# timdestan/go-raytracer

Hardware: AMD Instinct MI355X
Metric: Mrays/s (primary+shadow+reflect) at 4K depth=6; 1/2/4/8-GPU scaling (higher is better)
Workload: dtype f64; 1 GPU; c3: cylinder + cube + sphere (cone substitute) over a reflective plane, 4 lights, 3840x2160, depth 6; width=3840, height=2160, depth=6, lights=4, objects=4, parallelism=rows1-interleaved, frames_in_flight=2, schedule=auto, kernel=specialised, accel=bvh+cull

## Files before the change

### go-raytracer_amd/csrc/rt_kernel.hip

```cpp
#pragma clang fp contract(off)

#include <hip/hip_runtime.h>

#include <dlfcn.h>
#include <errno.h>
#include <fcntl.h>
#include <hip/hiprtc.h>
#include <sys/syscall.h>
#include <sys/wait.h>
#include <unistd.h>

#include <algorithm>
#include <atomic>
#include <chrono>
#include <condition_variable>
#include <cstdlib>
#include <functional>
#include <thread>
#include <cmath>
#include <array>
#include <cstdio>
#include <utility>
#include <cstring>
#include <limits>
// ... 1253 lines not shown
const char* rt_last_error(void) { return g_err.c_str(); }

int rt_create(int device, rt_context** out) {
  if (!out) return fail(RT_E_INVALID, "rt_create: out is NULL");
  *out = nullptr;
  if (device < 0) HIP_TRY(hipGetDevice(&device));
  int ndev = 0;
  HIP_TRY(hipGetDeviceCount(&ndev));
  if (device >= ndev) return fail(RT_E_INVALID, "rt_create: device index out of range");
  DeviceGuard guard(device);
  rt_context* c = new rt_context();
  c->device = device;
  hipDeviceProp_t prop;
  if (hipGetDeviceProperties(&prop, device) != hipSuccess) {
    delete c;
    return fail(RT_E_DEVICE, "hipGetDeviceProperties failed");
  }
  c->cus = prop.multiProcessorCount;
  c->lds_per_cu = (int)prop.maxSharedMemoryPerMultiProcessor;
  c->lds_per_block = (int)prop.sharedMemPerBlock;
  int per_cu = 0;
  if (hipOccupancyMaxActiveBlocksPerMultiprocessor(&per_cu, k_kernels[kernel_index(true, false, false, false, false)], WG, LDS_MAX_BYTES) !=
          hipSuccess || per_cu <= 0)
    per_cu = 2;
  c->grid_lds = c->cus * std::min(per_cu, 8);
  per_cu = 0;
  if (hipOccupancyMaxActiveBlocksPerMultiprocessor(&per_cu, k_kernels[kernel_index(false, false, false, false, false)], WG, 0) != hipSuccess ||
      per_cu <= 0)
    per_cu = 2;
  c->grid_glb = c->cus * std::min(per_cu, 8);
  std::vector<uint64_t> jump(JUMP_ENTRIES * 4);
  {
    typedef unsigned __int128 u128;
    const u128 mul = ((u128)2549297995355413924ULL << 64) | 4865540595714422341ULL;
    const u128 inc = ((u128)6364136223846793005ULL << 64) | 1442695040888963407ULL;
    u128 A = 1, Cc = 0;
    for (int step = 0; step < 2 * JUMP_ENTRIES; step++) {
      if (step % 2 == 0) {
        const int e = step / 2;
        jump[e * 4 + 0] = (uint64_t)(A >> 64);
        jump[e * 4 + 1] = (uint64_t)A;
        jump[e * 4 + 2] = (uint64_t)(Cc >> 64);
        jump[e * 4 + 3] = (uint64_t)Cc;
      }
      A = A * mul;
      Cc = Cc * mul + inc;
    }
  }
  int rc = upload(&c->jump, jump);
  if (rc == RT_OK && hipMalloc((void**)&c->queue, 2 * QSET_ALLOC * sizeof(unsigned int)) != hipSuccess)
    rc = fail(RT_E_NOMEM, "queue alloc");
  if (rc == RT_OK && hipMemset(c->queue, 0, 2 * QSET_ALLOC * sizeof(unsigned int)) != hipSuccess)
    rc = fail(RT_E_DEVICE, "queue memset");
  if (rc == RT_OK && hipMalloc((void**)&c->stats, sizeof(unsigned long long) * 64) != hipSuccess)
    rc = fail(RT_E_NOMEM, "stats alloc");
  if (rc == RT_OK && hipMemset(c->stats, 0, sizeof(unsigned long long) * 64) != hipSuccess)
    rc = fail(RT_E_DEVICE, "stats memset");
  c->stats_parts = c->cus * 8;
  if (rc == RT_OK && hipMalloc((void**)&c->stats_part, sizeof(unsigned long long) * STATS_PART * c->stats_parts) != hipSuccess)
    rc = fail(RT_E_NOMEM, "stats alloc");
  if (rc == RT_OK && hipMemset(c->stats_part, 0, sizeof(unsigned long long) * STATS_PART * c->stats_parts) != hipSuccess)
    rc = fail(RT_E_DEVICE, "stats memset");
  if (rc == RT_OK && (hipEventCreate(&c->ev0) != hipSuccess || hipEventCreate(&c->ev1) != hipSuccess))
    rc = fail(RT_E_DEVICE, "event create");
  if (rc != RT_OK) {
    rt_destroy(c);
    return rc;
  }
  *out = c;
  return RT_OK;
}

void rt_destroy(rt_context* c) {
  if (!c) return;
  DeviceGuard guard(c->device);
  free_scene(c->sc);
  (void)hipFree(c->ssim_buf);
  (void)hipFree(c->jump);
  (void)hipFree(c->queue);
  (void)hipFree(c->stats);
  (void)hipFree(c->stats_part);
  (void)hipFree(c->stack);
  (void)hipFree(c->vm_global);
  clear_orders(c);
  (void)hipFree(c->est);
  (void)hipFree(c->est_stats);
  (void)hipFree(c->gboard);
  (void)hipFree(c->gring);
  (void)hipFree(c->gctl);
  (void)hipFree(c->trace_ws);
  (void)hipFree(c->trace_ticket);
  (void)hipFree(c->cam_buf);
  (void)hipFree(c->cam_adapt);
  if (c->ev0) (void)hipEventDestroy(c->ev0);
  if (c->ev1) (void)hipEventDestroy(c->ev1);
  delete c;
}

static int launch(rt_context* c, int y0, int y1, int trow0, int stride, int ntrows, void* d_rgba, void* stream,
                  bool est);
static int estimate_costs(rt_context* c);
static bool want_order(const rt_context* c);
static int scene_install(rt_context* c, DevScene& s, const std::vector<uint32_t>* costs);

int rt_set_scene(rt_context* c, const rt_scene* in) {
  if (!c || !in) return fail(RT_E_INVALID, "rt_set_scene: NULL argument");
  if (in->width <= 1 || in->height <= 1) return fail(RT_E_INVALID, "rt_set_scene: width/height must be > 1");
  if (in->exp_mode < RT_EXP_AMD64_FMA || in->exp_mode > RT_EXP_PORTABLE)
    return fail(RT_E_INVALID, "rt_set_scene: unknown exp_mode");
// ... 813 lines not shown
      P.bvh_hi[k] = s.bvh_hi[k];
    }
  }

  if (c->launched && st != c->last_stream) HIP_TRY(hipStreamWaitEvent(st, c->ev1, 0));
  c->last_stream = st;
  c->launched = true;
  if (!est) HIP_TRY(hipEventRecord(c->ev0, st));
  const char* blob = s.blob;
  void* args[] = {(void*)&blob, (void*)&P};
  if (spec)
    HIP_TRY(hipModuleLaunchKernel(spec, grid, 1, 1, WG, 1, 1, shmem, st, args, nullptr));
  else
    HIP_TRY(hipLaunchKernel(kfn, dim3(grid), dim3(WG), args, shmem, st));
  HIP_TRY(hipGetLastError());
  c->qset ^= 1;
  HIP_TRY(hipEventRecord(c->ev1, st));
  if (est) return RT_OK;
  c->timed = true;
  c->last_spec = spec != nullptr;
  uint64_t rows = 0;
  if (stride > 0) {
    for (int j = 0; j < ntrows; j++) {
      int r0 = (trow0 + j * stride) * TILE;
      rows += (uint64_t)std::max(0, std::min((int)TILE, s.height - r0));
    }
  } else {
    rows = (uint64_t)(y1 - y0);
  }
  c->primary_pending += (uint64_t)4 * (uint64_t)s.width * rows;
  return RT_OK;
}

static bool want_order(const rt_context* c) {
  static const int env = rt_getenv("RT_TILE_ORDER") ? atoi(rt_getenv("RT_TILE_ORDER")) : 1;
  const DevScene& s = c->sc;
  return env != 0 && c->order_on && s.nobj > 0 && (scene_in_lds(s) || (env == 2 && s.use_bvh));
}

static int estimate_costs(rt_context* c) {
  clear_orders(c);
  if (!want_order(c)) return RT_OK;
  const DevScene& s = c->sc;
  DeviceGuard guard(c->device);
  const size_t n = (size_t)((s.width + TILE - 1) / TILE) * ((s.height + TILE - 1) / TILE);
  if (n > c->est_cap) {
    (void)hipFree(c->est);
    c->est = nullptr;
    c->est_cap = 0;
    HIP_TRY(hipMalloc((void**)&c->est, n * sizeof(unsigned int)));
    c->est_cap = n;
  }
  if (!c->est_stats) {
    HIP_TRY(hipMalloc((void**)&c->est_stats, sizeof(unsigned long long) * 64));
    HIP_TRY(hipMemset(c->est_stats, 0, sizeof(unsigned long long) * 64));
  }
  const auto t0 = std::chrono::steady_clock::now();
  HIP_TRY(hipMemset(c->est, 0, n * sizeof(unsigned int)));
  int rc = launch(c, 0, s.height, 0, 0, 0, nullptr, nullptr, true);
  if (rc != RT_OK) return rc;
  std::vector<uint32_t> cost(n);
  HIP_TRY(hipMemcpy(cost.data(), c->est, n * sizeof(unsigned int), hipMemcpyDeviceToHost));
  unsigned long long wd = 0;
  HIP_TRY(hipMemcpy(&wd, c->est_stats + ST_WATCHDOG, sizeof wd, hipMemcpyDeviceToHost));
  HIP_TRY(hipMemset(c->est_stats, 0, sizeof(unsigned long long) * 64));
  if (wd) return fail(RT_E_DEVICE, "render watchdog in the tile-cost estimate (kernel bug)");
  c->tile_cost.swap(cost);
  c->order_ms = std::chrono::duration<double, std::milli>(std::chrono::steady_clock::now() - t0).count();
  c->timed = false;
  return RT_OK;
}

int rt_set_work_sharing(rt_context* c, int enable) {
  if (!c) return fail(RT_E_INVALID, "rt_set_work_sharing: NULL context");
  if (enable < 0 || enable > RT_SHARE_AUTO) return fail(RT_E_INVALID, "rt_set_work_sharing: unknown mode");
  c->share_mode = enable;
  return c->has_scene ? spec_prepare(c) : RT_OK;
}

int rt_set_tile_order(rt_context* c, int enable) {
  if (!c) return fail(RT_E_INVALID, "rt_set_tile_order: NULL context");
  c->order_on = enable != 0;
  if (!c->has_scene) return RT_OK;
  if (!c->order_on) {
    clear_orders(c);
    return RT_OK;
  }
  return c->tile_cost.empty() ? estimate_costs(c) : RT_OK;
}

int rt_tile_order_info(rt_context* c, int* active, double* estimate_ms) {
  if (!c || !active || !estimate_ms) return fail(RT_E_INVALID, "rt_tile_order_info: NULL argument");
  *active = c->tile_cost.empty() ? 0 : 1;
  *estimate_ms = c->order_ms;
  return RT_OK;
}

int rt_render_rows_async(rt_context* c, int y0, int y1, void* d_rgba, void* stream) {
  if (!c || !c->has_scene) return fail(RT_E_INVALID, "rt_render_rows_async: no scene set");
  if (!d_rgba) return fail(RT_E_INVALID, "rt_render_rows_async: NULL output");
  if (y0 < 0 || y1 > c->sc.height || y1 <= y0) return fail(RT_E_INVALID, "rt_render_rows_async: bad row range");
  return launch(c, y0, y1, 0, 0, 0, d_rgba, stream, false);
}

int rt_render_tile_rows_async(rt_context* c, int trow0, int trow_stride, int ntrows, void* d_rgba, void* stream) {
  if (!c || !c->has_scene) return fail(RT_E_INVALID, "rt_render_tile_rows_async: no scene set");
  if (!d_rgba) return fail(RT_E_INVALID, "rt_render_tile_rows_async: NULL output");
  if (trow0 < 0 || trow_stride <= 0 || ntrows <= 0) return fail(RT_E_INVALID, "rt_render_tile_rows_async: bad tile rows");
  return launch(c, 0, c->sc.height, trow0, trow_stride, ntrows, d_rgba, stream, false);
}


int rt_read_stats(rt_context* c, void* stream, int reset, rt_stats* out) {
  if (!c || !out) return fail(RT_E_INVALID, "rt_read_stats: NULL argument");
  DeviceGuard guard(c->device);
  hipStream_t st = (hipStream_t)stream;
  unsigned long long h[ST_COUNT] = {}, wd = 0;
  std::vector<unsigned long long> part((size_t)STATS_PART * c->stats_parts);
  HIP_TRY(hipMemcpyAsync(part.data(), c->stats_part, part.size() * sizeof(unsigned long long), hipMemcpyDeviceToHost, st));
  HIP_TRY(hipMemcpyAsync(&wd, c->stats + ST_WATCHDOG, sizeof wd, hipMemcpyDeviceToHost, st));
  HIP_TRY(hipStreamSynchronize(st));
  for (int b = 0; b < c->stats_parts; b++)
    for (int k = 0; k < ST_COUNT; k++) h[k] += part[(size_t)b * STATS_PART + k];
  if (wd) {
    HIP_TRY(hipMemsetAsync(c->stats, 0, sizeof(unsigned long long) * 64, st));
    HIP_TRY(hipMemsetAsync(c->stats_part, 0, part.size() * sizeof(unsigned long long), st));
    c->gslots = 0;
    HIP_TRY(hipStreamSynchronize(st));
    c->primary_pending = 0;
    c->launches = 0;
    return fail(RT_E_DEVICE, "render watchdog: " + std::to_string(wd) + " waves stopped unfinished (kernel bug)");
  }
  std::memset(out, 0, sizeof *out);
  uint64_t per_kind[RT_NUM_KINDS] = {0, 0, 0, 0, 0};
  if (c->has_scene)
    for (int k : c->sc.kinds) per_kind[k]++;
  out->primary_rays = c->primary_pending;
  out->secondary_rays = h[ST_TRACED] - c->primary_pending;
  out->shadow_rays = h[ST_SHADOW];
  for (int k = 0; k < RT_NUM_KINDS; k++) {
    out->tests[k] = h[ST_TRACED] * per_kind[k];
    out->shadow_tests[k] = h[ST_STESTS + k];
  }
  out->shaded_hits = h[ST_SHADED];
  out->surface_errors = h[ST_SURFERR];
#ifdef RT_PHASE_TIMING
  {
    unsigned long long ph[N_PHASE];
    HIP_TRY(hipMemcpy(ph, c->stats + ST_PHASE, sizeof ph, hipMemcpyDeviceToHost));
    unsigned long long tot = 0;
    for (int k = 0; k < N_PHASE; k++) tot += ph[k];
    if (tot) {
      static const char* nm[N_PHASE] = {"refill", "gen", "trace_loop", "trace_unwind", "shade_surface",
                                        "light_dirs", "shadow_loops", "lighting", "material", "shade_unwind"};
      fprintf(stderr, "[phase]");
      for (int k = 0; k < N_PHASE; k++) fprintf(stderr, " %s=%.3f", nm[k], (double)ph[k] / (double)tot);
      fprintf(stderr, " total_wave_cycles=%.4g\n", (double)tot);
      unsigned long long bd[8];
      HIP_TRY(hipMemcpy(bd, c->stats + ST_BVHDIAG, sizeof bd, hipMemcpyDeviceToHost));
      if (c->wdiag && c->last_waves > 0) {
        std::vector<unsigned long long> w((size_t)c->last_waves * 4);
        HIP_TRY(hipMemcpy(w.data(), c->wdiag, w.size() * sizeof(unsigned long long), hipMemcpyDeviceToHost));
        std::vector<std::pair<unsigned long long, int>> life;
        for (int i = 0; i < c->last_waves; i++) life.push_back({w[(size_t)i * 4], i});
        std::sort(life.begin(), life.end());
        auto pct = [&](double q) { return (double)life[std::min(life.size() - 1, (size_t)(q * life.size()))].first; };
        fprintf(stderr, "[tail] lifetime p10 %.4g p50 %.4g p90 %.4g p99 %.4g max %.4g;", pct(0.1), pct(0.5), pct(0.9),
                pct(0.99), (double)life.back().first);
        for (int k = 1; k <= 4 && k <= (int)life.size(); k++) {
          const int i = life[life.size() - k].second;
          fprintf(stderr, " [life %.4g chunks %llu last-chunk %.4g]", (double)w[(size_t)i * 4], w[(size_t)i * 4 + 1],
                  (double)w[(size_t)i * 4 + 2]);
        }
        double lc = 0;
        for (int i = 0; i < c->last_waves; i++) lc += (double)w[(size_t)i * 4 + 2];
        fprintf(stderr, " mean last-chunk %.4g\n", lc / c->last_waves);
      }
#ifdef RT_CSG_DIAG
      {
        unsigned long long cd[8] = {0, 0, 0, 0, 0, 0, 0, 0};
        if (hipMemcpyFromSymbol(cd, HIP_SYMBOL(g_csg_diag), sizeof cd) == hipSuccess && cd[0]) {
          fprintf(stderr, "[csg] searches %llu, register-list overflows %llu (%.2f%%), mean live leaves %.2f\n", cd[0],
                  cd[1], 100.0 * cd[1] / cd[0], (double)cd[2] / cd[0]);
          if (cd[6])
            fprintf(stderr,
                    "[csg] group visits %llu: leaf-major iterations %llu (lanes %.1f of 64), lane-major %llu (lanes "
                    "%.1f), lane-leaf candidates %llu\n",
                    cd[6], cd[3], cd[3] ? (double)cd[5] / cd[3] : 0.0, cd[4], cd[4] ? (double)cd[5] / cd[4] : 0.0, cd[5]);
        }
      }
#endif
      {
        unsigned long long sh[6];
        HIP_TRY(hipMemcpy(sh, c->stats + ST_SHDIAG, sizeof sh, hipMemcpyDeviceToHost));
        fprintf(stderr, "[share] posted samples %llu subtrees %llu, claims %llu, reclaims %llu, waits %llu, idle polls %llu\n",
                sh[0], sh[1], sh[2], sh[3], sh[4], sh[5]);
      }
      {
        unsigned long long pd[6];
        HIP_TRY(hipMemcpy(pd, c->stats + ST_PASSDIAG, sizeof pd, hipMemcpyDeviceToHost));
        fprintf(stderr, "[passes] trace %llu (%.1f lanes), shade %llu (%.1f lanes), gen %llu (%.1f lanes)\n", pd[0],
                (double)pd[1] / std::max(1ull, pd[0]), pd[2], (double)pd[3] / std::max(1ull, pd[2]), pd[4],
                (double)pd[5] / std::max(1ull, pd[4]));
        unsigned long long ld[2];
        HIP_TRY(hipMemcpy(ld, c->stats + ST_LANEDIAG, sizeof ld, hipMemcpyDeviceToHost));
        fprintf(stderr, "[lanes] rounds %llu, lanes waiting in S_DONE (finished quad / pair samples) %.2f per round\n", ld[1],
                (double)ld[0] / (double)std::max(1ull, ld[1]));
      }
      unsigned long long steps = 0;
      HIP_TRY(hipMemcpy(&steps, c->stats + ST_CLOCKSTEP, sizeof steps, hipMemcpyDeviceToHost));
      const double nw = std::max(1.0, (double)c->last_waves * c->launches - (double)steps);
      fprintf(stderr, "[waves] lifetime mean %.4g cycles, max %.4g cycles (mean/max %.3f; %llu waves with a clock step left out)\n",
              (double)bd[6] / nw, (double)bd[7], (double)bd[6] / nw / (double)std::max(1ull, bd[7]), steps);
      if (bd[4] + bd[5])
        fprintf(stderr, "[bvh] wave traversals trace=%llu shadow=%llu; nodes/traversal trace=%.1f shadow=%.1f; "
                        "leaves/traversal trace=%.1f shadow=%.1f\n", bd[4], bd[5], (double)bd[0] / (double)std::max(1ull, bd[4]),
                (double)bd[1] / (double)std::max(1ull, bd[5]), (double)bd[2] / (double)std::max(1ull, bd[4]),
                (double)bd[3] / (double)std::max(1ull, bd[5]));
#ifdef RT_EXACT_DIAG
      unsigned long long ex[2 * RT_NUM_KINDS + 2];
      HIP_TRY(hipMemcpy(ex, c->stats + ST_EXDIAG, sizeof ex, hipMemcpyDeviceToHost));
      fprintf(stderr, "[exact] lane tests after culling per kind (trace/shadow):");
      for (int k = 0; k < RT_NUM_KINDS; k++) fprintf(stderr, " k%d=%llu/%llu", k, ex[2 * k], ex[2 * k + 1]);
      fprintf(stderr, "; wave batches trace=%llu shadow=%llu\n", ex[2 * RT_NUM_KINDS], ex[2 * RT_NUM_KINDS + 1]);
#endif
    }
  }
#endif
  float ms = 0.f;
  if (c->timed && hipEventElapsedTime(&ms, c->ev0, c->ev1) == hipSuccess) out->kernel_ms = ms;
  out->devices = 1;
  out->device_kernel_ms[0] = out->kernel_ms;
  if (reset) {
    HIP_TRY(hipMemsetAsync(c->stats, 0, sizeof(unsigned long long) * 64, st));
    HIP_TRY(hipMemsetAsync(c->stats_part, 0, part.size() * sizeof(unsigned long long), st));
    HIP_TRY(hipStreamSynchronize(st));
    c->primary_pending = 0;
    c->launches = 0;
  }
  return RT_OK;
}

int rt_last_kernel_ms(rt_context* c, double* ms_out) {
  if (!c || !ms_out) return fail(RT_E_INVALID, "rt_last_kernel_ms: NULL argument");
  if (!c->timed) return fail(RT_E_INVALID, "rt_last_kernel_ms: nothing rendered yet");
  DeviceGuard guard(c->device);
  HIP_TRY(hipEventSynchronize(c->ev1));
  float ms = 0.f;
  HIP_TRY(hipEventElapsedTime(&ms, c->ev0, c->ev1));
  *ms_out = ms;
  return RT_OK;
}

int rt_debug_run_surface(rt_context* c, int program, int n, const long long* face, const double* u,
                         const double* v, double* out10, int* err) {
  if (!c || !c->has_scene || n <= 0 || !face || !u || !v || !out10 || !err)
    return fail(RT_E_INVALID, "rt_debug_run_surface: bad arguments");
  if (program < 0 || program >= c->sc.num_programs) return fail(RT_E_INVALID, "rt_debug_run_surface: no such program");
  DeviceGuard guard(c->device);
  long long* df = nullptr;
  double *du = nullptr, *dv = nullptr, *dout = nullptr;
  int* derr = nullptr;
  int rc = RT_OK;
  if (hipMalloc((void**)&df, n * sizeof(long long)) != hipSuccess || hipMalloc((void**)&du, n * sizeof(double)) != hipSuccess ||
      hipMalloc((void**)&dv, n * sizeof(double)) != hipSuccess ||
      hipMalloc((void**)&dout, (size_t)n * 10 * sizeof(double)) != hipSuccess ||
      hipMalloc((void**)&derr, n * sizeof(int)) != hipSuccess)
    rc = fail(RT_E_NOMEM, "rt_debug_run_surface: alloc");
  if (rc == RT_OK && (hipMemcpy(df, face, n * sizeof(long long), hipMemcpyHostToDevice) != hipSuccess ||
                      hipMemcpy(du, u, n * sizeof(double), hipMemcpyHostToDevice) != hipSuccess ||
                      hipMemcpy(dv, v, n * sizeof(double), hipMemcpyHostToDevice) != hipSuccess))
    rc = fail(RT_E_DEVICE, "rt_debug_run_surface: copy");
  if (rc == RT_OK) {
    hipLaunchKernelGGL(rt_debug_vm_kernel, dim3((n + 63) / 64), dim3(64), 0, nullptr, (const char*)c->sc.blob,
                       c->sc.off_code, c->sc.off_consts, c->sc.off_entry, program, df, du, dv, dout, derr, n);
    if (hipGetLastError() != hipSuccess || hipDeviceSynchronize() != hipSuccess)
      rc = fail(RT_E_DEVICE, "rt_debug_run_surface: launch");
  }
  if (rc == RT_OK && (hipMemcpy(out10, dout, (size_t)n * 10 * sizeof(double), hipMemcpyDeviceToHost) != hipSuccess ||
                      hipMemcpy(err, derr, n * sizeof(int), hipMemcpyDeviceToHost) != hipSuccess))
    rc = fail(RT_E_DEVICE, "rt_debug_run_surface: copy back");
  (void)hipFree(df);
  (void)hipFree(du);
  (void)hipFree(dv);
  (void)hipFree(dout);
  (void)hipFree(derr);
  return rc;
// ... 11 lines not shown
```

### go-raytracer_amd/csrc/rt_render.h

```cpp
#pragma once
#pragma clang fp contract(off)

#ifndef __HIPCC_RTC__
#include <hip/hip_runtime.h>
#endif

#include "rt_abi.h"
#include "rt_device.h"

#ifndef RT_CULL
#define RT_CULL 1
#endif
#ifndef RT_SHARE
#define RT_SHARE 0
#endif
#ifndef RT_PAIRS
#define RT_PAIRS 0
#endif
#ifndef RT_FAR_SHIFT
#define RT_FAR_SHIFT 1
#endif
#ifndef RT_GS_POLL
#define RT_GS_POLL 3
#endif
#ifndef RT_GS_HELPERS
#define RT_GS_HELPERS 16
#endif
#ifndef RT_SHADE_NUM
#define RT_SHADE_NUM 3
#endif
#ifndef RT_SHADE_DEN
#define RT_SHADE_DEN 4
#endif
#ifdef RT_COST_MAP
#undef RT_SHARE
#define RT_SHARE 0
#endif

#define CULL_AND(a, b) (bool)((int)(bool)(a) & (int)(bool)(b))

using namespace rt;

enum { SF_VM = 1, SF_LDIR = 2, SF_LSPOT = 4 };
#ifdef RT_SPEC_NOBJ
constexpr int spec_kinds[RT_SPEC_NOBJ] = {RT_SPEC_KINDS};
constexpr int spec_kind_mask() {
  int m = 0;
  for (int i = 0; i < RT_SPEC_NOBJ; i++) m |= 1 << spec_kinds[i];
  return m;
}
constexpr int SPEC_KMASK = spec_kind_mask();
constexpr int SPEC_FEAT = RT_SPEC_FEAT;
static_assert(SPEC_KMASK == RT_SPEC_KMASK, "RT_SPEC_KINDS and RT_SPEC_KMASK disagree");
#elif defined(RT_SPEC_KMASK)
constexpr int SPEC_KMASK = RT_SPEC_KMASK;
constexpr int SPEC_FEAT = RT_SPEC_FEAT;
#else
constexpr int SPEC_KMASK = -1;
constexpr int SPEC_FEAT = -1;
#endif
__device__ constexpr bool spec_kind(int k) { return ((SPEC_KMASK >> k) & 1) != 0; }
__device__ constexpr bool spec_feat(int f) { return (SPEC_FEAT & f) != 0; }

enum { GEO = 16, SHD = 32, MAT = 16, LGT = 16, OMAT = 8, GLOB = 16 };
enum { FRAME_FIELDS = 15, CORE = 5, EXT_ROWS = 6, FR_EXT = 3, FR_COL = 11, FR_REFL = 14 };
enum { CHUNK = 64, TILE = 8, WG = 256, WAVES_PER_WG = WG / 64 };
enum { QHEADS = 8 , QSTRIDE = 16  };
static_assert(QHEADS >= 1 && QHEADS <= 32, "QHEADS");
enum { QSTEAL = 1 };
enum { QSET = QHEADS * QSTRIDE ,
       QSET_ALLOC = 32 * QSTRIDE  };
enum { QCHUNK_PIXEL = 64 };
enum { SCH = 32 };
enum { SHADOW_CHECK = 8 };
enum { ST_SHADOW = 0, ST_TRACED = 1, ST_SHADED = 2, ST_SURFERR = 3, ST_STESTS = 4, ST_COUNT = ST_STESTS + RT_NUM_KINDS,
       ST_PHASE = 16, N_PHASE = 10, ST_BVHDIAG = 26, ST_EXDIAG = 34, ST_SHDIAG = 48, ST_PASSDIAG = 54,
       ST_CLOCKSTEP = 60, ST_LANEDIAG = 61 ,
       ST_WATCHDOG = 63,
       STATS_PART = 16  };
enum { SH_POST_S = 0, SH_POST_T = 1, SH_CLAIM = 2, SH_RECLAIM = 3, SH_WAIT = 4, SH_SPIN = 5 };
#ifdef RT_PHASE_TIMING
#define SHDIAG(k) atomicAdd(P.stats + ST_SHDIAG + (k), 1ull)
#else
#define SHDIAG(k) (void)0
#endif
enum { S_IDLE = 0, S_TRACE = 1, S_SHADE = 2, S_DONE = 3 };
enum { LDS_MAX_BYTES = 40 * 1024 };
enum { JUMP_ENTRIES = 20 * 4 };

__device__ __forceinline__ int est_x(int pts, unsigned int k) { return pts == 1 ? TILE / 2 : 2 + 4 * (int)(k & 1u); }
__device__ __forceinline__ int est_y(int pts, unsigned int k) { return pts == 1 ? TILE / 2 : 2 + 4 * (int)((k >> 1) & 1u); }

struct Params {
  int lds_frames_off;
  int lds_levels;
  int lds_full;
  int lds_ext_off;
  int stream_off;
  int qmask_off;
  int jump_off;
  int off_geo, off_shade, off_mats, off_lights, off_kind, off_objmat, off_pref, off_csg, off_code, off_consts,
      off_entry, blob_bytes;
  int lds_vm_off;
  double* vm_global;
  const uint64_t* jump;
  unsigned int* queue;
  unsigned int* queue_next;
  unsigned long long* stats;
  unsigned long long* stats_part;
  unsigned long long* wdiag;
  double* stack;
  uint32_t* out;
  int width, height, depth, nobj, nlights, y0, y1, tiles_x;
  int trow0, trow_stride;
  unsigned int total_slots;
  int frames;
  const float* bvh_nodes;
  const double* bvh_geo;
  const int* planes;
  int nplanes, bvh_stack_off;
  double bvh_lo[3], bvh_hi[3];
  const int* runs;
  int nruns;
  const double* arec;
  const double* urec;
  int cnt_off;
  int kind_mask;
  int board_off;
  uint64_t* gboard;
  uint64_t* gring;
  uint64_t* gctl;
// ... 1297 lines not shown
      pk = lane_ < min(SCH, P.nobj - c0) ? S.kind[c0 + lane_] : 0;
    };
    auto store = [&]() {
#pragma unroll
      for (int q = 0; q < PER; q++) dst[lane_ + q * 64] = pre[q];
      if (lane_ < SCH) skind[lane_] = pk;
      __builtin_amdgcn_fence(__ATOMIC_SEQ_CST, "wavefront");
    };
    if (P.nobj <= 0) return;
    fetch(0);
    store();
    for (int c0 = 0; c0 < P.nobj; c0 += SCH) {
      const int n = min(SCH, P.nobj - c0);
      const bool more = c0 + SCH < P.nobj;
      if (more) fetch(c0 + SCH);
      for (int j = 0; j < n; j++)
        if (!body(c0 + j, skind[j], sbuf + (size_t)j * GEO)) return;
      __builtin_amdgcn_fence(__ATOMIC_SEQ_CST, "wavefront");
      if (more) store();
    }
  };
  const d3 eye = mk(0.0, 0.0, -1.0);

  int state = S_IDLE;
  bool need_gen = false;
  int px = 0, py = 0, sample = 0, sp = 0;
  unsigned int pout = 0;
  uint32_t held_px = ~0u, held_val = 0u;
  auto flush_pixels = [&]() {
    if (held_px != ~0u) P.out[held_px] = held_val;
    held_px = ~0u;
  };
  constexpr bool WAVE_SGPR = BVH || CSG;
  const int wave = WAVE_SGPR ? __builtin_amdgcn_readfirstlane((int)(threadIdx.x >> 6)) : (int)(threadIdx.x >> 6);
  int my_idle = 0, spins = 0;
  bool my_active = true;
  bool sh_live = false;
  int hit_i = 0, hit_f = 0;
  double hit_t = 0.0;
  Pcg rng{0, 0};
  d3 sum = mk(0, 0, 0);
  d3 sum2 = mk(0, 0, 0);
  Ray ray;
  ray.o = mk(0, 0, 0);
  ray.d = mk(0, 0, 1);

  unsigned int pool_next = 0, pool_end = 0;
  int qhead = 0;
  bool exhausted = false;
  unsigned long long* cnt = reinterpret_cast<unsigned long long*>(smem + P.cnt_off);
  unsigned long long* kcnt = reinterpret_cast<unsigned long long*>(smem + P.cnt_off + CNT_KIND_OFF);
  for (int k = 0; k < RT_NUM_KINDS; k++) kcnt[k * WG + threadIdx.x] = 0;
  constexpr bool CNT_REMAT = BVH || CSG;
  auto opaque_s = [](uint32_t b) {
    b = (uint32_t)__builtin_amdgcn_readfirstlane((int)b);
    asm volatile("" : "+s"(b));
    return b;
  };
  auto cnt_kind = [&](int k, uint64_t v) {
    if constexpr (CNT_REMAT) {
      uint32_t l;
      asm volatile("v_mbcnt_lo_u32_b32 %0, -1, 0\n\tv_mbcnt_hi_u32_b32 %0, -1, %0" : "=v"(l));
      const uint32_t a = opaque_s((uint32_t)P.cnt_off + (uint32_t)(CNT_KIND_OFF + (k * WG + wave * 64) * 8)) + l * 8u;
      atomicAdd(reinterpret_cast<unsigned long long*>(smem + a), (unsigned long long)v);
    } else {
      atomicAdd(&kcnt[k * WG + threadIdx.x], (unsigned long long)v);
    }
  };
  auto cnt_unit = [&](int k, bool b) {
    const unsigned int n = (unsigned int)__popcll(wave_ballot(b));
    if (lane == 0 && n) {
      if constexpr (CNT_REMAT)
        atomicAdd(reinterpret_cast<unsigned long long*>(
                      smem + opaque_s((uint32_t)P.cnt_off + (uint32_t)((k * WAVES_PER_WG + wave) * 8))),
                  (unsigned long long)n);
      else
        atomicAdd(&cnt[k * WAVES_PER_WG + wave], (unsigned long long)n);
    }
  };
  WaveStack bst;
  bst.mask = reinterpret_cast<uint64_t*>(smem + P.bvh_stack_off) + (threadIdx.x >> 6) * BVH_STACK;
  bst.ref = reinterpret_cast<int*>(smem + P.bvh_stack_off + WAVES_PER_WG * BVH_STACK * 8) + (threadIdx.x >> 6) * BVH_STACK;
#ifdef RT_PHASE_TIMING
  uint64_t ph_acc[N_PHASE] = {0, 0, 0, 0, 0, 0, 0, 0, 0, 0};
  uint64_t bd_tnodes = 0, bd_snodes = 0, bd_tleaf = 0, bd_sleaf = 0, bd_trays = 0, bd_srays = 0;
  uint64_t pd_tr = 0, pd_trl = 0, pd_sh = 0, pd_shl = 0, pd_gen = 0, pd_genl = 0;
  uint64_t ld_done = 0, ld_rounds = 0;
#ifdef RT_COST_MAP
  uint32_t lane_cost = 0;
#endif
#endif

  const double W1 = (double)(P.width - 1), H1 = (double)(P.height - 1);

  auto gen_ray = [&]() {
    double dx = pcg_float64(rng) - 0.5;
    double dy = pcg_float64(rng) - 0.5;
    const double vw = G[9], vh = G[10];
    double u = ((double)px + dx) / W1 * vw - vw / 2.0;
    double v = ((double)py + dy) / H1 * vh - vh / 2.0;
    ray.o = mk(u, -v, 0.0);
    ray.d = norm(sub(ray.o, eye));
  };

  auto sample_rng = [&](int x, int y, int k) {
    const int ry = y % 20;
    const uint64_t* j = P.jump + (ry * 4 + k) * 4;
    return pcg_jump(Pcg{0xDEADULL ^ (uint64_t)x, 0xBEEFULL ^ (uint64_t)(y - ry)}, j[0], j[1], j[2], j[3]);
  };
  auto wait_slot = [&]() -> int {
    if (RT_SHARE == 1 && !QD && sp == 0) return lw_fork(Bd->lw[threadIdx.x], sample);
    return PK_SLOT_OF(__double_as_longlong(core_ld(sp - 1, 4)));
  };
  auto advance_sample = [&](uint32_t w) {
    for (;;) {
      if (P.est_out && sample == 1) {
        state = S_IDLE;
        return;
      }
      if (PR && sample == ((lane & 1) ? 4 : 2)) {
        state = S_DONE;
        return;
      }
      if (sample == 4) {
        d3 c = scale(sum, 1.0 / 4.0);
        uint32_t r8 = go_f64_to_u32(c.x * 65535.0) >> 8;
        uint32_t g8 = go_f64_to_u32(c.y * 65535.0) >> 8;
        uint32_t b8 = go_f64_to_u32(c.z * 65535.0) >> 8;
#ifdef RT_COST_MAP
        P.out[pout] = lane_cost;
        lane_cost = 0;
#else
        const uint32_t v = (r8 & 0xffu) | ((g8 & 0xffu) << 8) | ((b8 & 0xffu) << 16) | 0xff000000u;
        held_px = pout;
        held_val = v;
#endif
        state = S_IDLE;
        return;
      }
      if (RT_SHARE != 1 || __builtin_expect(sample < lw_own_end(w), 1)) {
        need_gen = true;
        state = S_TRACE;
        return;
      }
      const int q = lw_fork(w, sample);
      if (board_reclaim(Bd, q)) {
        SHDIAG(SH_RECLAIM);
        board_free(Bd, q);
        Bd->lw[threadIdx.x] = (w & ~7u) | (uint32_t)(sample + 1);
        rng = sample_rng(px, py, sample);
        need_gen = true;
        state = S_TRACE;
        return;
      }
      if (!board_done(Bd, q)) {
        SHDIAG(SH_WAIT);
        state = S_WAIT;
        return;
      }
      sum = add(sum, board_take(Bd, q));
      sample++;
    }
  };

  auto unwind = [&](bool have_res, d3 res, bool pf_valid, long long pf_packed, d3 pf_lw, double pf_kr) {
    while (wave_any(have_res)) {
      if (have_res) {
        if (sp == 0) {
          if constexpr (QD) {
            sum = res;
            state = S_DONE;
          } else {
            if (PR && (lane & 1))
              (sample == 2 ? sum : sum2) = res;
            else
              sum = add(sum, res);
            sample++;
            state = S_ADV;
          }
          have_res = false;
        } else {
          double* f = frame_ptr(stk, sp - 1);
          long long packed;
          if (pf_valid)
            packed = pf_packed;
          else
            packed = __double_as_longlong(core_ld(sp - 1, 4));
          int fl = (int)(packed & 0xff);
          if (RT_SHARE && __builtin_expect((fl & FL_TASK) != 0, 0)) {
            if constexpr (RT_SHARE == 2)
              gs_deliver(P.gboard, PK_SLOT_OF(packed), res);
            else
              board_deliver(Bd, PK_SLOT_OF(packed), res);
            sp = 0;
            state = S_IDLE;
            have_res = false;
          } else if ((fl & FL_HASR) && (fl & FL_HAST) && !(fl & FL_STAGE)) {
            double* e = ext(sp - 1);
            const d3 first = res;
            bool here = true;
            core_st(sp - 1, 4, __longlong_as_double(packed | FL_STAGE));
            if (RT_SHARE && __builtin_expect((fl & FL_FORKED) != 0, 0)) {
              const int q = PK_SLOT_OF(packed);
              if (RT_SHARE == 2 ? gs_reclaim(P.gboard, q) : board_reclaim(Bd, q)) {
                SHDIAG(SH_RECLAIM);
                if (RT_SHARE == 1) board_free(Bd, q);
              } else if (RT_SHARE == 2 ? gs_done(P.gboard, q) : board_done(Bd, q)) {
                here = false;
                res = RT_SHARE == 2 ? gs_take(P.gboard, q) : board_take(Bd, q);
              } else {
                SHDIAG(SH_WAIT);
                here = false;
                state = S_WAIT;
                have_res = false;
              }
            }
            if (here) {
              ray.o = ld3(e, 0);
              ray.d = ld3(e, 3);
              state = S_TRACE;
              have_res = false;
            }
            st3(e, 0, first);
          } else {
            const double* FM = S.mats + (size_t)(packed >> PK_MAT) * MAT;
            d3 R = mk(0, 0, 0), Tr = mk(0, 0, 0);
            if ((fl & FL_HASR) && (fl & FL_HAST)) {
              R = ld3(ext(sp - 1), 0);
              Tr = res;
            } else if (fl & FL_HASR) {
              R = res;
            } else {
              Tr = res;
            }
            d3 lw;
            double kr;
            if (pf_valid) {
              lw = pf_lw;
              kr = pf_kr;
            } else {
              lw = mk(core_ld(sp - 1, 0), core_ld(sp - 1, 1), core_ld(sp - 1, 2));
              kr = core_ld(sp - 1, 3);
            }
            d3 fcol;
            double frefl;
            if (spec_feat(SF_VM) && (fl & FL_VMMAT)) {
              fcol = ld3(f, FR_COL);
              frefl = f[FR_REFL * 64];
            } else {
              fcol = mk(FM[0], FM[1], FM[2]);
              frefl = FM[3];
            }
            res = combine((fl & FL_TMODE) != 0, lw, fcol, frefl, kr, R, Tr);
            sp--;
          }
          pf_valid = false;
        }
      }
    }
  };

  PH_BEGIN();
#ifdef RT_PHASE_TIMING
  const uint64_t life_t0 = ph_t0_;
  uint64_t last_grab = life_t0, nchunk_taken = 0;
#endif
  uint32_t guard_iters = 0;
  for (;;) {
    if (++guard_iters > (1u << 26)) {
      if (lane == 0) atomicAdd(P.stats + ST_WATCHDOG, 1ull);
      break;
    }
    if constexpr (!QD) {
      if (wave_any(state == S_ADV)) {
        if (wave_any(state == S_ADV && held_px != ~0u && (RT_SHARE || (!PR && sample == 4)))) flush_pixels();
        if (state == S_ADV) {
          const uint32_t w = RT_SHARE == 1 ? Bd->lw[threadIdx.x] : 4u;
          if (RT_SHARE == 1 && __builtin_expect(lw_task(w) >= 0, 0)) {
            board_deliver(Bd, lw_task(w), sum);
            Bd->lw[threadIdx.x] = 0u;
            state = S_IDLE;
          } else {
            advance_sample(w);
          }
        }
      }
    }
    if constexpr (QD) {
      const uint64_t dn = wave_ballot(state == S_DONE);
      const uint64_t qd = dn & (dn >> 1) & (dn >> 2) & (dn >> 3) & 0x1111111111111111ull;
      if (qd) {
        d3 sm = add(mk(0, 0, 0), sum);
#pragma unroll
        for (int k = 1; k < 4; k++) {
          const int lk = (lane + k) & 63;
          sm = add(sm, mk(__shfl(sum.x, lk), __shfl(sum.y, lk), __shfl(sum.z, lk)));
        }
        if (wave_any(((qd >> lane) & 1) && held_px != ~0u)) flush_pixels();
        if ((qd >> lane) & 1) {
          const d3 c = scale(sm, 1.0 / 4.0);
          const uint32_t r8 = go_f64_to_u32(c.x * 65535.0) >> 8;
          const uint32_t g8 = go_f64_to_u32(c.y * 65535.0) >> 8;
          const uint32_t b8 = go_f64_to_u32(c.z * 65535.0) >> 8;
          const uint32_t v = (r8 & 0xffu) | ((g8 & 0xffu) << 8) | ((b8 & 0xffu) << 16) | 0xff000000u;
          held_px = pout;
          held_val = v;
        }
        if ((qd >> (lane & ~3)) & 1) state = S_IDLE;
      }
    }
    if constexpr (PR) {
      const uint64_t dn = wave_ballot(state == S_DONE);
      const uint64_t pd = dn & (dn >> 1) & 0x5555555555555555ull;
      if (pd) {
        const int lb = (lane + 1) & 63;
        const d3 c2 = mk(__shfl(sum.x, lb), __shfl(sum.y, lb), __shfl(sum.z, lb));
        const d3 c3 = mk(__shfl(sum2.x, lb), __shfl(sum2.y, lb), __shfl(sum2.z, lb));
        const d3 sm = add(add(sum, c2), c3);
        if (wave_any(((pd >> lane) & 1) && held_px != ~0u)) flush_pixels();
        if ((pd >> lane) & 1) {
          const d3 c = scale(sm, 1.0 / 4.0);
          const uint32_t r8 = go_f64_to_u32(c.x * 65535.0) >> 8;
          const uint32_t g8 = go_f64_to_u32(c.y * 65535.0) >> 8;
          const uint32_t b8 = go_f64_to_u32(c.z * 65535.0) >> 8;
          const uint32_t v = (r8 & 0xffu) | ((g8 & 0xffu) << 8) | ((b8 & 0xffu) << 16) | 0xff000000u;
          held_px = pout;
          held_val = v;
        }
        if ((pd >> (lane & ~1)) & 1) state = S_IDLE;
      }
    }
    for (;;) {
      const uint64_t il = wave_ballot(state == S_IDLE);
      const uint64_t mask = QD   ? il & (il >> 1) & (il >> 2) & (il >> 3) & 0x1111111111111111ull
                            : PR ? il & (il >> 1) & 0x5555555555555555ull
                                 : il;
      const bool need = ((mask >> (QD ? (lane & ~3) : PR ? (lane & ~1) : lane)) & 1) != 0;
      if (mask == 0 || exhausted) break;
      if (pool_next >= pool_end) {
        const unsigned int nchunks = (P.total_slots + QCHUNK - 1) / QCHUNK;
        unsigned int c = nchunks;
        const int nheads = gridDim.x >= QHEADS ? min(QHEADS, QSTEAL + 1) : QHEADS;
        while (qhead < nheads) {
          const unsigned int h = (blockIdx.x + qhead) % QHEADS;
          const unsigned int dm = __builtin_amdgcn_readfirstlane(__atomic_load_n(qdrained, __ATOMIC_RELAXED));
          if ((dm >> h) & 1u) {
            qhead++;
            continue;
          }
          unsigned int n = 0;
          if (lane == 0) n = atomicAdd(P.queue + h * QSTRIDE, 1u);
          c = __builtin_amdgcn_readfirstlane(n) * QHEADS + h;
          if (c < nchunks) break;
          if (lane == 0) atomicOr(qdrained, 1u << h);
          qhead++;
        }
        if (qhead >= nheads) {
          exhausted = true;
          break;
        }
#ifdef RT_PHASE_TIMING
        last_grab = stamp();
        nchunk_taken++;
#endif
        pool_next = c * QCHUNK;
        pool_end = min(pool_next + (unsigned int)QCHUNK, P.total_slots);
      }
      const unsigned int rank = QD   ? (unsigned int)__popcll(mask & ((1ull << (lane & ~3)) - 1ull))
                                : PR ? (unsigned int)__popcll(mask & ((1ull << (lane & ~1)) - 1ull))
                                     : __builtin_amdgcn_mbcnt_hi((unsigned int)(mask >> 32),
                                                                 __builtin_amdgcn_mbcnt_lo((unsigned int)mask, 0u));
      unsigned int take = min((unsigned int)__popcll(mask), pool_end - pool_next);
      if (!QD && !PR && P.est_out) {
        if (need && rank < take) {
          const unsigned int u = pool_next + rank, t = u / (unsigned)P.est_pts, k = u % (unsigned)P.est_pts;
          px = min((int)(t % (unsigned)P.tiles_x) * TILE + est_x(P.est_pts, k), P.width - 1);
          py = min((int)(t / (unsigned)P.tiles_x) * TILE + est_y(P.est_pts, k), P.y1 - 1);
          pout = t;
          const int ry = py % 20;
          rng = pcg_jump(Pcg{0xDEADULL ^ (uint64_t)px, 0xBEEFULL ^ (uint64_t)(py - ry)}, jrows[ry * 4],
                         jrows[ry * 4 + 1], jrows[ry * 4 + 2], jrows[ry * 4 + 3]);
          sample = 0;
          if (RT_SHARE == 1) Bd->lw[threadIdx.x] = 1u;
          sum = mk(0, 0, 0);
          sp = 0;
          need_gen = true;
          state = S_TRACE;
        }
        pool_next += take;
        continue;
      }
      unsigned int tile = pool_next / (TILE * TILE);
      if (P.order) tile = P.order[tile];
      const int trow = (int)(tile / (unsigned)P.tiles_x);
      const int x0 = (int)((tile % (unsigned)P.tiles_x) * TILE);
      const int orow0 = trow * TILE;
      const int y0t = P.trow_stride > 0 ? (P.trow0 + trow * P.trow_stride) * TILE : P.y0 + orow0;
      const int r0t = y0t % 20;
      if (need && rank < take) {
        const unsigned int within = pool_next % (TILE * TILE) + rank;
        const int tx = QD ? (int)(((within >> 4) & 1u) * 4u + (within & 3u)) : (int)(within % TILE);
        const int ty = QD ? (int)((within >> 5) * 4u + ((within >> 2) & 3u)) : (int)(within / TILE);
        const int x = x0 + tx;
        const int orow = orow0 + ty;
        const int y = y0t + ty;
        if (x < P.width && y < P.y1) {
          px = x;
          py = y;
          pout = (unsigned int)orow * (unsigned int)P.width + (unsigned int)x;
          const int ry = r0t + ty >= 20 ? r0t + ty - 20 : r0t + ty;
          const int ymin = y - ry;
          Pcg s0{0xDEADULL ^ (uint64_t)x, 0xBEEFULL ^ (uint64_t)ymin};
          sample = QD ? (lane & 3) : PR ? (lane & 1) * 2 : 0;
          const uint64_t* j = (QD || PR) ? P.jump + (ry * 4 + sample) * 4 : jrows + ry * 4;
          rng = pcg_jump(s0, j[0], j[1], j[2], j[3]);
          sum = mk(0, 0, 0);
          sp = 0;
          if (RT_SHARE == 1) Bd->lw[threadIdx.x] = 4u;
          need_gen = true;
          state = S_TRACE;
        }
      }
      pool_next += take;
    }
    if (RT_SHARE == 1 && !sh_live && !exhausted && (guard_iters & 3u) == 0u)
      sh_live = __builtin_amdgcn_readfirstlane(__hip_atomic_load(&Bd->nidle, __ATOMIC_RELAXED, RT_WG_SCOPE)) > 0;
    if (RT_SHARE == 2 && !sh_live && !exhausted && (guard_iters & 7u) == 0u)
      sh_live = __builtin_amdgcn_readfirstlane(lane == 0 ? (int)gs_ld32(g_nidle) : 0) > 0;
    if (RT_SHARE && !sh_live && exhausted) sh_live = true;
    if (RT_SHARE && !sh_live) {
    } else if constexpr (RT_SHARE == 2) {
      auto rfl64 = [](uint64_t v) {
        return ((uint64_t)(uint32_t)__builtin_amdgcn_readfirstlane((int)(v >> 32)) << 32) |
               (uint32_t)__builtin_amdgcn_readfirstlane((int)v);
      };
      if (__builtin_expect(wave_any(state == S_WAIT), 0)) {
        if (state == S_WAIT && gs_done(P.gboard, wait_slot())) state = S_RESUME;
      }
      if (gs_helper || (guard_iters & (unsigned)RT_GS_POLL) == 0u) {
        int nid = 0;
        uint64_t gh = 0, gt = 0;
        if (lane == 0) {
          gt = gs_ld(g_tail);
          if (!gs_helper || (guard_iters & 7u) == 0u || gt != gs_t) {
            nid = (int)gs_ld32(g_nidle);
            gh = gs_ld(g_head);
          } else {
            nid = gs_nid;
            gh = gs_h;
          }
        }
        gs_nid = __builtin_amdgcn_readfirstlane(nid);
        gs_h = rfl64(gh);
        gs_t = rfl64(gt);
      }
      const int nid = gs_nid;
      const uint64_t gh = gs_h, gt = gs_t;
      const long long outstanding = (long long)(gt - gh);
      const int want = nid - (int)min(outstanding, (long long)(1 << 30));
      if (__builtin_expect(want > 0 && outstanding < GS_RSH / 2, 0)) {
        const bool busy_lane = state == S_TRACE || state == S_SHADE || state == S_WAIT;
        int L = -1;
        if (busy_lane)
          for (int l = min(sp - 1, P.depth - 1 - GS_MIN_LEVELS); l >= 0; l--) {
            const int f = (int)(__double_as_longlong(core_ld(l, 4)) & 0xff);
            if (f & FL_TASK) break;
            if ((f & (FL_HASR | FL_HAST | FL_STAGE | FL_FORKED)) == (FL_HASR | FL_HAST)) L = l;
          }
        const uint64_t cm = wave_ballot(L >= 0);
        if (cm) {
          const int npost = min((int)__popcll(cm), want);
          const int rk = (int)__builtin_amdgcn_mbcnt_hi((unsigned int)(cm >> 32),
                                                        __builtin_amdgcn_mbcnt_lo((unsigned int)cm, 0u));
          const bool post = L >= 0 && rk < npost;
          int q = 0;
          if (post) {
            SHDIAG(SH_POST_T);
// ... 451 lines not shown
#endif
          if (r & 7) {
#ifdef RT_PHASE_TIMING
            bd_tleaf++;
#endif
            const int first = r >> 3, count = r & 7;
            for (int j = first; j < first + count; j++) {
              const LeafRec L = ld_leaf(P.bvh_geo, j);
              const float tmax = found ? (float)(best_t - bt0) * 1.0001f + 1e-4f : 3.0e38f;
              const bool test = may_hit_s(act, bof, df, tmax, L.cx, L.cy, L.cz, L.cr, bslack);
              if (!wave_any(test)) continue;
              trace_exact(L.i, L.k, L.R.m, test);
            }
          } else {
            const cfptr nb = (cfptr)P.bvh_nodes + (size_t)(r >> 3) * BN;
            const ciptr ni = (ciptr)(nb + 12);
            const float tmax = found ? (float)(best_t - bt0) * 1.0001f + 1e-4f : 3.0e38f;
            float t0 = 0.0f, t1 = 0.0f;
            const bool a0 = may_hit_box_a(act, bof, idf, bslack, tmax, nb, t0);
            const bool a1 = may_hit_box_a(act, bof, idf, bslack, tmax, nb + 6, t1);
            const uint64_t m0 = wave_ballot(a0), m1 = wave_ballot(a1);
            const bool c1_first = 2 * __popcll(wave_ballot(a0 && a1 && t1 < t0)) > __popcll(m0 & m1);
            bvh_next(bst, ssp, lane, c1_first, ni[0], ni[1], m0, m1, nr, nm, have);
          }
        }
      }
      cnt_unit(CNT_TRACED, tr);
#ifdef RT_PHASE_TIMING
      pd_tr++;
      pd_trl += (uint64_t)__popcll(wave_ballot(tr));
#endif
      if (!QD && P.est_out && tr) atomicAdd(P.est_out + pout, 1u);
      PH_MARK(2);
      d3 res = mk(0, 0, 0);
      if (tr) {
        if (found) {
          state = S_SHADE;
          hit_i = best_i;
          hit_f = best_f;
          hit_t = best_t;
        } else {
          double t = 0.5 * (ray.d.y + 1.0);
          res = lerp(mk(G[3], G[4], G[5]), mk(G[6], G[7], G[8]), t);
        }
      }
      const bool resumed = RT_SHARE && state == S_RESUME;
      if (__builtin_expect(resumed, 0))
        res = RT_SHARE == 2 ? gs_take(P.gboard, wait_slot()) : board_take(Bd, wait_slot());
      unwind((tr && !found) || resumed, res, pf, pf_packed, pf_lw, pf_kr);
      PH_MARK(3);
    }

    const uint64_t nsh = popc_ballot(state == S_SHADE);
    const uint64_t ntr = popc_ballot(state == S_TRACE ||
                                     (!QD && state == S_ADV && (RT_SHARE || sample < (PR && !(lane & 1) ? 2 : 4))));
    if (nsh == 0 || (ntr != 0 && nsh * RT_SHADE_DEN < (nsh + ntr) * RT_SHADE_NUM)) continue;

    const bool hit = state == S_SHADE;
    cnt_unit(CNT_SHADED, hit);
#ifdef RT_PHASE_TIMING
    pd_sh++;
    pd_shl += (uint64_t)__popcll(wave_ballot(hit));
#endif
    d3 pw = mk(0, 0, 0), nw = mk(0, 0, 1);
    int mat = 0;
    bool surf_bad = false;
    if (hit) {
      int si = hit_i, sf = hit_f;
      bool flip = false;
      if constexpr (CSG) {
        if (S.kind[hit_i] == RT_CSG) {
          const int* ci = reinterpret_cast<const int*>(S.geo + (size_t)hit_i * GEO + 14);
          si = P.nobj + ci[0] + (hit_f >> 4);
          flip = ((hit_f >> 3) & 1) != 0;
          sf = hit_f & 7;
        }
      }
      const double* g = S.geo + (size_t)si * GEO;
      const double* s = S.shade + (size_t)si * SHD;
      const int k = S.kind[si];
      Ray l = to_obj(g, ray);
      d3 p = add(l.o, scale(l.d, hit_t));
      pw = mk(s[0] * p.x + s[1] * p.y + s[2] * p.z + s[3], s[4] * p.x + s[5] * p.y + s[6] * p.z + s[7],
              s[8] * p.x + s[9] * p.y + s[10] * p.z + s[11]);
      if (spec_kind(RT_SPHERE) && k == RT_SPHERE) {
        nw = p;
      } else if ((spec_kind(RT_CYLINDER) && k == RT_CYLINDER) || (spec_kind(RT_CONE) && k == RT_CONE)) {
        d3 n = sf == 0 ? (k == RT_CONE ? mk(p.x, -p.y, p.z) : mk(p.x, 0, p.z)) : (sf == 1 ? mk(0, 1, 0) : mk(0, -1, 0));
        nw = norm(mk(g[0] * n.x + g[4] * n.y + g[8] * n.z, g[1] * n.x + g[5] * n.y + g[9] * n.z,
                     g[2] * n.x + g[6] * n.y + g[10] * n.z));
      } else {
        nw = mk(s[12 + sf * 3], s[13 + sf * 3], s[14 + sf * 3]);
      }
      if (flip) nw = neg(nw);
      mat = S.objmat[(size_t)si * OMAT + sf];
      if (spec_feat(SF_VM) && mat < 0) {
        double u, v;
        bool bad = false;
        long long face = (k == RT_PLANE) ? 0 : sf;
        if (k == RT_SPHERE) {
          bad = __builtin_fabs(p.y) > 1;
          v = (p.y + 1.0) / 2.0;
          u = go_acos(p.z / __builtin_sqrt(1.0 - p.y * p.y)) / 6.283185307179586;
        } else if ((k == RT_CYLINDER || k == RT_CONE) && sf == 0) {
          u = (go_atan2(p.x, p.z) + 3.141592653589793) / 6.283185307179586;
          v = p.y;
        } else {
          u = p.x;
// ... 563 lines not shown
```

Measured before the change: 73220 Mrays/s.

## Advance to next sample inside unwind for BVH kernels, skipping the ADV round

For BVH-specialised kernels, a finished sample now moves straight to generating the next sample inside the unwind loop instead of going through the S_ADV state and the round head. The unwind of reflect/transmit frames is also simplified to pass the result through unless transmit mode is set. The aim is fewer wave round-trips through the refill/advance logic and less divergence between lanes at different sample counts. Phase-timing stats move to a larger stats buffer with two new phases. This risks changed pixel flush logic and correctness for the PR/share modes.

```diff
diff --git a/go-raytracer_amd/csrc/rt_kernel.hip b/go-raytracer_amd/csrc/rt_kernel.hip
--- a/go-raytracer_amd/csrc/rt_kernel.hip
+++ b/go-raytracer_amd/csrc/rt_kernel.hip
@@ -1329,9 +1329,9 @@
     rc = fail(RT_E_NOMEM, "queue alloc");
   if (rc == RT_OK && hipMemset(c->queue, 0, 2 * QSET_ALLOC * sizeof(unsigned int)) != hipSuccess)
     rc = fail(RT_E_DEVICE, "queue memset");
-  if (rc == RT_OK && hipMalloc((void**)&c->stats, sizeof(unsigned long long) * 64) != hipSuccess)
+  if (rc == RT_OK && hipMalloc((void**)&c->stats, sizeof(unsigned long long) * ST_TOTAL) != hipSuccess)
     rc = fail(RT_E_NOMEM, "stats alloc");
-  if (rc == RT_OK && hipMemset(c->stats, 0, sizeof(unsigned long long) * 64) != hipSuccess)
+  if (rc == RT_OK && hipMemset(c->stats, 0, sizeof(unsigned long long) * ST_TOTAL) != hipSuccess)
     rc = fail(RT_E_DEVICE, "stats memset");
   c->stats_parts = c->cus * 8;
   if (rc == RT_OK && hipMalloc((void**)&c->stats_part, sizeof(unsigned long long) * STATS_PART * c->stats_parts) != hipSuccess)
@@ -2251,8 +2251,8 @@
     c->est_cap = n;
   }
   if (!c->est_stats) {
-    HIP_TRY(hipMalloc((void**)&c->est_stats, sizeof(unsigned long long) * 64));
-    HIP_TRY(hipMemset(c->est_stats, 0, sizeof(unsigned long long) * 64));
+    HIP_TRY(hipMalloc((void**)&c->est_stats, sizeof(unsigned long long) * ST_TOTAL));
+    HIP_TRY(hipMemset(c->est_stats, 0, sizeof(unsigned long long) * ST_TOTAL));
   }
   const auto t0 = std::chrono::steady_clock::now();
   HIP_TRY(hipMemset(c->est, 0, n * sizeof(unsigned int)));
@@ -2262,7 +2262,7 @@
   HIP_TRY(hipMemcpy(cost.data(), c->est, n * sizeof(unsigned int), hipMemcpyDeviceToHost));
   unsigned long long wd = 0;
   HIP_TRY(hipMemcpy(&wd, c->est_stats + ST_WATCHDOG, sizeof wd, hipMemcpyDeviceToHost));
-  HIP_TRY(hipMemset(c->est_stats, 0, sizeof(unsigned long long) * 64));
+  HIP_TRY(hipMemset(c->est_stats, 0, sizeof(unsigned long long) * ST_TOTAL));
   if (wd) return fail(RT_E_DEVICE, "render watchdog in the tile-cost estimate (kernel bug)");
   c->tile_cost.swap(cost);
   c->order_ms = std::chrono::duration<double, std::milli>(std::chrono::steady_clock::now() - t0).count();
@@ -2322,7 +2322,7 @@
   for (int b = 0; b < c->stats_parts; b++)
     for (int k = 0; k < ST_COUNT; k++) h[k] += part[(size_t)b * STATS_PART + k];
   if (wd) {
-    HIP_TRY(hipMemsetAsync(c->stats, 0, sizeof(unsigned long long) * 64, st));
+    HIP_TRY(hipMemsetAsync(c->stats, 0, sizeof(unsigned long long) * ST_TOTAL, st));
     HIP_TRY(hipMemsetAsync(c->stats_part, 0, part.size() * sizeof(unsigned long long), st));
     c->gslots = 0;
     HIP_TRY(hipStreamSynchronize(st));
@@ -2350,10 +2350,11 @@
     unsigned long long tot = 0;
     for (int k = 0; k < N_PHASE; k++) tot += ph[k];
     if (tot) {
-      static const char* nm[N_PHASE] = {"refill", "gen", "trace_loop", "trace_unwind", "shade_surface",
-                                        "light_dirs", "shadow_loops", "lighting", "material", "shade_unwind"};
+      static const char* nm[N_PHASE] = {"round_head", "gen", "trace_loop", "trace_unwind", "shade_surface",
+                                        "light_dirs", "shadow_loops", "lighting", "material", "shade_unwind",
+                                        "sample_adv", "refill_deal"};
       fprintf(stderr, "[phase]");
-      for (int k = 0; k < N_PHASE; k++) fprintf(stderr, " %s=%.3f", nm[k], (double)ph[k] / (double)tot);
+      for (int k = 0; k < N_PHASE; k++) fprintf(stderr, " %s=%.4f", nm[k], (double)ph[k] / (double)tot);
       fprintf(stderr, " total_wave_cycles=%.4g\n", (double)tot);
       unsigned long long bd[8];
       HIP_TRY(hipMemcpy(bd, c->stats + ST_BVHDIAG, sizeof bd, hipMemcpyDeviceToHost));
@@ -2431,7 +2432,7 @@
   out->devices = 1;
   out->device_kernel_ms[0] = out->kernel_ms;
   if (reset) {
-    HIP_TRY(hipMemsetAsync(c->stats, 0, sizeof(unsigned long long) * 64, st));
+    HIP_TRY(hipMemsetAsync(c->stats, 0, sizeof(unsigned long long) * ST_TOTAL, st));
     HIP_TRY(hipMemsetAsync(c->stats_part, 0, part.size() * sizeof(unsigned long long), st));
     HIP_TRY(hipStreamSynchronize(st));
     c->primary_pending = 0;
diff --git a/go-raytracer_amd/csrc/rt_render.h b/go-raytracer_amd/csrc/rt_render.h
--- a/go-raytracer_amd/csrc/rt_render.h
+++ b/go-raytracer_amd/csrc/rt_render.h
@@ -74,9 +74,10 @@
 enum { SCH = 32 };
 enum { SHADOW_CHECK = 8 };
 enum { ST_SHADOW = 0, ST_TRACED = 1, ST_SHADED = 2, ST_SURFERR = 3, ST_STESTS = 4, ST_COUNT = ST_STESTS + RT_NUM_KINDS,
-       ST_PHASE = 16, N_PHASE = 10, ST_BVHDIAG = 26, ST_EXDIAG = 34, ST_SHDIAG = 48, ST_PASSDIAG = 54,
+       ST_BVHDIAG = 26, ST_EXDIAG = 34, ST_SHDIAG = 48, ST_PASSDIAG = 54,
        ST_CLOCKSTEP = 60, ST_LANEDIAG = 61 ,
        ST_WATCHDOG = 63,
+       ST_PHASE = 64, N_PHASE = 12, ST_TOTAL = ST_PHASE + N_PHASE ,
        STATS_PART = 16  };
 enum { SH_POST_S = 0, SH_POST_T = 1, SH_CLAIM = 2, SH_RECLAIM = 3, SH_WAIT = 4, SH_SPIN = 5 };
 #ifdef RT_PHASE_TIMING
@@ -1480,6 +1481,7 @@
   unsigned long long* kcnt = reinterpret_cast<unsigned long long*>(smem + P.cnt_off + CNT_KIND_OFF);
   for (int k = 0; k < RT_NUM_KINDS; k++) kcnt[k * WG + threadIdx.x] = 0;
   constexpr bool CNT_REMAT = BVH || CSG;
+  constexpr bool ADV_UNW = BVH;
   auto opaque_s = [](uint32_t b) {
     b = (uint32_t)__builtin_amdgcn_readfirstlane((int)b);
     asm volatile("" : "+s"(b));
@@ -1510,7 +1512,7 @@
   bst.mask = reinterpret_cast<uint64_t*>(smem + P.bvh_stack_off) + (threadIdx.x >> 6) * BVH_STACK;
   bst.ref = reinterpret_cast<int*>(smem + P.bvh_stack_off + WAVES_PER_WG * BVH_STACK * 8) + (threadIdx.x >> 6) * BVH_STACK;
 #ifdef RT_PHASE_TIMING
-  uint64_t ph_acc[N_PHASE] = {0, 0, 0, 0, 0, 0, 0, 0, 0, 0};
+  uint64_t ph_acc[N_PHASE] = {0, 0, 0, 0, 0, 0, 0, 0, 0, 0, 0, 0};
   uint64_t bd_tnodes = 0, bd_snodes = 0, bd_tleaf = 0, bd_sleaf = 0, bd_trays = 0, bd_srays = 0;
   uint64_t pd_tr = 0, pd_trl = 0, pd_sh = 0, pd_shl = 0, pd_gen = 0, pd_genl = 0;
   uint64_t ld_done = 0, ld_rounds = 0;
@@ -1546,11 +1548,11 @@
         state = S_IDLE;
         return;
       }
-      if (PR && sample == ((lane & 1) ? 4 : 2)) {
+      if (PR && (ADV_UNW || sample == ((lane & 1) ? 4 : 2))) {
         state = S_DONE;
         return;
       }
-      if (sample == 4) {
+      if ((ADV_UNW && RT_SHARE != 1) || sample == 4) {
         d3 c = scale(sum, 1.0 / 4.0);
         uint32_t r8 = go_f64_to_u32(c.x * 65535.0) >> 8;
         uint32_t g8 = go_f64_to_u32(c.y * 65535.0) >> 8;
@@ -1592,22 +1594,31 @@
   };
 
   auto unwind = [&](bool have_res, d3 res, bool pf_valid, long long pf_packed, d3 pf_lw, double pf_kr) {
+#define FINISH_SAMPLE() \
+  do { \
+      if constexpr (QD) { \
+        sum = res;  \
+        state = S_DONE; \
+      } else { \
+        if (PR && (lane & 1)) \
+          (sample == 2 ? sum : sum2) = res; \
+        else \
+          sum = add(sum, res); \
+        sample++; \
+        if (!ADV_UNW || RT_SHARE == 1 || (PR ? !(sample & 1) : sample == 4) || (P.est_out && sample == 1)) { \
+          state = S_ADV; \
+        } else { \
+          need_gen = true; \
+          state = S_TRACE; \
+        } \
+      } \
+      have_res = false; \
+  } while (0)
     while (wave_any(have_res)) {
       if (have_res) {
-        if (sp == 0) {
-          if constexpr (QD) {
-            sum = res;
-            state = S_DONE;
-          } else {
-            if (PR && (lane & 1))
-              (sample == 2 ? sum : sum2) = res;
-            else
-              sum = add(sum, res);
-            sample++;
-            state = S_ADV;
-          }
-          have_res = false;
-        } else {
+        if (!ADV_UNW && sp == 0) {
+          FINISH_SAMPLE();
+        } else if (!ADV_UNW || sp != 0) {
           double* f = frame_ptr(stk, sp - 1);
           long long packed;
           if (pf_valid)
@@ -1653,7 +1664,18 @@
           } else {
             const double* FM = S.mats + (size_t)(packed >> PK_MAT) * MAT;
             d3 R = mk(0, 0, 0), Tr = mk(0, 0, 0);
-            if ((fl & FL_HASR) && (fl & FL_HAST)) {
+            if constexpr (ADV_UNW) {
+              R = res;
+              Tr = res;
+              if (fl & FL_TMODE) {
+                if ((fl & FL_HASR) && (fl & FL_HAST))
+                  R = ld3(ext(sp - 1), 0);
+                else if (fl & FL_HASR)
+                  Tr = mk(0, 0, 0);
+                else
+                  R = mk(0, 0, 0);
+              }
+            } else if ((fl & FL_HASR) && (fl & FL_HAST)) {
               R = ld3(ext(sp - 1), 0);
               Tr = res;
             } else if (fl & FL_HASR) {
@@ -1684,9 +1706,11 @@
           }
           pf_valid = false;
         }
+        if (ADV_UNW && have_res && sp == 0) FINISH_SAMPLE();
       }
     }
   };
+#undef FINISH_SAMPLE
 
   PH_BEGIN();
 #ifdef RT_PHASE_TIMING
@@ -1699,6 +1723,7 @@
       if (lane == 0) atomicAdd(P.stats + ST_WATCHDOG, 1ull);
       break;
     }
+    PH_MARK(0);
     if constexpr (!QD) {
       if (wave_any(state == S_ADV)) {
         if (wave_any(state == S_ADV && held_px != ~0u && (RT_SHARE || (!PR && sample == 4)))) flush_pixels();
@@ -1758,6 +1783,7 @@
         if ((pd >> (lane & ~1)) & 1) state = S_IDLE;
       }
     }
+    PH_MARK(10);
     for (;;) {
       const uint64_t il = wave_ballot(state == S_IDLE);
       const uint64_t mask = QD   ? il & (il >> 1) & (il >> 2) & (il >> 3) & 0x1111111111111111ull
@@ -1851,6 +1877,7 @@
       }
       pool_next += take;
     }
+    PH_MARK(11);
     if (RT_SHARE == 1 && !sh_live && !exhausted && (guard_iters & 3u) == 0u)
       sh_live = __builtin_amdgcn_readfirstlane(__hip_atomic_load(&Bd->nidle, __ATOMIC_RELAXED, RT_WG_SCOPE)) > 0;
     if (RT_SHARE == 2 && !sh_live && !exhausted && (guard_iters & 7u) == 0u)
@@ -2408,8 +2435,10 @@
     }
 
     const uint64_t nsh = popc_ballot(state == S_SHADE);
-    const uint64_t ntr = popc_ballot(state == S_TRACE ||
-                                     (!QD && state == S_ADV && (RT_SHARE || sample < (PR && !(lane & 1) ? 2 : 4))));
+    const uint64_t ntr =
+        ADV_UNW ? popc_ballot(state == S_TRACE || (!QD && RT_SHARE && state == S_ADV))
+                : popc_ballot(state == S_TRACE ||
+                              (!QD && state == S_ADV && (RT_SHARE || sample < (PR && !(lane & 1) ? 2 : 4))));
     if (nsh == 0 || (ntr != 0 && nsh * RT_SHADE_DEN < (nsh + ntr) * RT_SHADE_NUM)) continue;
 
     const bool hit = state == S_SHADE;
```

After: 73250 Mrays/s, median of 4. No clear change (+0.0%).
